# joeyee/Onet

Hardware: AMD Instinct MI355X
Metric: training images/sec (twin 256x256 pass) (higher is better)
Workload: dtype f32

## Files before the change

### onet_amd/_lib.py

```python
from __future__ import annotations

import ctypes
import os
import re

HERE = os.path.dirname(os.path.abspath(__file__))
HEADER = os.path.join(os.path.dirname(HERE), "include", "onet_hip.h")
EVAL_HEADER = os.path.join(os.path.dirname(HERE), "include", "onet_hip_eval.h")
RAGGED_HEADER = os.path.join(os.path.dirname(HERE), "include", "onet_hip_ragged.h")
RAGGED_SPLIT_HEADER = os.path.join(os.path.dirname(HERE), "include", "onet_hip_ragged_split.h")
ANYMAP_HEADER = os.path.join(os.path.dirname(HERE), "include", "onet_hip_anymap.h")
PAIRS_HEADER = os.path.join(os.path.dirname(HERE), "include", "onet_hip_pairs.h")
UPMAP_HEADER = os.path.join(os.path.dirname(HERE), "include", "onet_hip_upmap.h")
SPLIT_PAIRS_HEADER = os.path.join(os.path.dirname(HERE), "include", "onet_hip_split_pairs.h")
OPTIM_HEADER = os.path.join(os.path.dirname(HERE), "include", "onet_hip_optim.h")
LIBPATH = os.environ.get("ONET_HIP_LIB") or os.path.join(HERE, "libonet_hip.so")

_CT = {
    "int": ctypes.c_int,
    "int64_t": ctypes.c_int64,
    "uint64_t": ctypes.c_uint64,
    "float": ctypes.c_float,
    "double": ctypes.c_double,
}


def parse_header(path: str = HEADER):
    src = open(path).read()
    src = re.sub(r"/\*.*?\*/", " ", src, flags=re.S)
    src = re.sub(r"//[^\n]*", " ", src)
# ... 26 lines not shown
_lib = None
_protos = None


def load(build_if_missing: bool = True):
    global _lib, _protos
    if _lib is not None:
        return _lib
    if not os.path.exists(LIBPATH):
        if not build_if_missing:
            raise OnetHipError(f"{LIBPATH} not built; run `python -m onet_amd.build`")
        from . import build as _build
        _build.build()
    lib = ctypes.CDLL(LIBPATH)
    _protos = {}
    for header in (HEADER, EVAL_HEADER, RAGGED_HEADER, RAGGED_SPLIT_HEADER, ANYMAP_HEADER, PAIRS_HEADER, UPMAP_HEADER, SPLIT_PAIRS_HEADER, OPTIM_HEADER):
        protos = parse_header(header)
        for name, (restype, argtypes, _) in protos.items():
            try:
                fn = getattr(lib, name)
            except AttributeError as e:
                raise OnetHipError(f"libonet_hip.so does not export {name} declared in {os.path.basename(header)}") from e
            fn.restype = restype
            fn.argtypes = argtypes
        _protos.update(protos)
    _lib = lib
    return lib


def last_error() -> str:
    return load().onet_last_error().decode()
# ... 16 lines not shown
```

### onet_amd/build.py

```python
import os
import subprocess
import sys

HERE = os.path.dirname(os.path.abspath(__file__))
CSRC = os.path.join(HERE, "csrc")
LIB = os.path.join(HERE, "libonet_hip.so")
SOURCES = ["abi.cpp", "conv_mfma.hip", "conv_wino4.hip", "conv_wino4w.hip", "conv_split.hip", "convt_gemm.hip", "stem.hip", "bn.hip", "spatial.hip", "head_loss.hip", "optim.hip", "evalside.hip", "clutter.hip"]
ARCH = "gfx950"


def _stale():
    if not os.path.exists(LIB):
        return True
    t = os.path.getmtime(LIB)
    deps = [os.path.join(CSRC, f) for f in os.listdir(CSRC) if f.endswith((".hip", ".cpp", ".hpp"))] + \
        [os.path.join(HERE, "..", "include", h) for h in ("onet_hip.h", "onet_hip_eval.h", "onet_hip_ragged.h", "onet_hip_ragged_split.h", "onet_hip_anymap.h", "onet_hip_pairs.h", "onet_hip_upmap.h", "onet_hip_split_pairs.h", "onet_hip_optim.h")]
    return any(os.path.getmtime(d) > t for d in deps)


def build(force=False, verbose=False, variant=None, flags=()):
    lib = LIB if variant is None else os.path.join(HERE, f"libonet_hip_{variant}.so")
    if variant is None and not force and not _stale():
        return LIB
    hipcc = os.environ.get("HIPCC", "/opt/rocm/bin/hipcc")
    objdir = CSRC if variant is None else os.path.join(CSRC, "_" + variant)
    os.makedirs(objdir, exist_ok=True)
    objs = []
    procs = []
    for src in SOURCES:
        obj = os.path.join(objdir, src.rsplit(".", 1)[0] + ".o")
        cmd = [hipcc, "-x", "hip", f"--offload-arch={ARCH}", "-O3", "-fPIC", "-std=c++17", "-Wall",
# ... 26 lines not shown
```

### onet_amd/csrc/conv_mfma.hip

```cpp
#include <algorithm>
#include <cstdlib>
#include "common.hpp"

using namespace onet;

typedef float f32x16 __attribute__((ext_vector_type(16)));

__global__ void pack3x3_kernel(const float* __restrict__ w, float* __restrict__ wf,
                               float* __restrict__ wd, int Cout, int Cin) {
    int64_t n = (int64_t)Cout * Cin * 9;
    for (int64_t i = blockIdx.x * (int64_t)blockDim.x + threadIdx.x; i < n;
         i += (int64_t)gridDim.x * blockDim.x) {
        int t = (int)(i % 9);
        int64_t r = i / 9;
        int ci = (int)(r % Cin), co = (int)(r / Cin);
        float v = w[i];
        if (wf) wf[((int64_t)ci * 9 + t) * Cout + co] = v;
        if (wd) wd[((int64_t)co * 9 + (8 - t)) * Cin + ci] = v;
    }
}

__global__ void packT2x2_kernel(const float* __restrict__ w, float* __restrict__ wf,
                                float* __restrict__ wd, float* __restrict__ wq, int Cin, int Cout) {
    int64_t n = (int64_t)Cin * Cout * 4;
// ... 465 lines not shown
            }
        }
        __syncthreads();
    }
    float* sl = a.slab + (int64_t)ks * TAPS * a.Cout * a.Cin;
    const int ci = ci0 + wn * 32 + l31;
    if (ci < a.Cin) {
#pragma unroll
        for (int t = 0; t < NTAP; ++t) {
#pragma unroll
            for (int r = 0; r < 16; ++r) {
                const int co = co0 + wm * 32 + (r & 3) + 8 * (r >> 2) + 4 * kh;
                if (co < a.Cout) sl[((int64_t)(tg * NTAP + t) * a.Cout + co) * a.Cin + ci] = acc[t][r];
            }
        }
    }
}

__global__ __launch_bounds__(256) void wgrad_reduce_kernel(const float* __restrict__ slab, float* __restrict__ dw,
                                                           int splitK, int taps, int Cout, int Cin, int out_layout,
                                                           int accumulate) {
    __shared__ float red[256];
    const int64_t n = (int64_t)Cout * Cin;
    const int t = blockIdx.y;
    const int64_t i = (int64_t)blockIdx.x * 64 + (threadIdx.x & 63);
    const int g = threadIdx.x >> 6;
    float s = 0.f;
    if (i < n)
        for (int k = g; k < splitK; k += 4) s += slab[((int64_t)k * taps + t) * n + i];
    red[threadIdx.x] = s;
// ... 4 lines not shown
        int64_t o;
        if (out_layout == 0) {
            o = i * taps + t;
        } else {
            const int Ct = Cout / 4, q = co / Ct, cot = co % Ct;
            o = ((int64_t)ci * Ct + cot) * 4 + q;
        }
        dw[o] = accumulate ? dw[o] + s : s;
    }
}

namespace onet {
int launch_wgrad_reduce(const float* slab, float* dw, int splitK, int taps, int Cout, int Cin, int out_layout, int accumulate,
                        hipStream_t st) {
    const int64_t n = (int64_t)Cout * Cin;
    hipLaunchKernelGGL(wgrad_reduce_kernel, dim3((unsigned)cdiv(n, 64), (unsigned)taps), dim3(256), 0, st, slab, dw, splitK,
                       taps, Cout, Cin, out_layout, accumulate);
    return check_launch("wgrad_reduce_kernel");
}
}

constexpr int STEM_ROWS = 32;
template <int CIN, int COG, bool BN = false>
__global__ __launch_bounds__(256) void conv3x3_stem_wgrad_kernel(WgArgs a) {
    constexpr int NV = COG * CIN * 9;
    __shared__ float red[4][NV];
    const int cogs = (a.Cout + COG - 1) / COG;
    const int bandsY = (a.H + STEM_ROWS - 1) / STEM_ROWS;
    const int cg = blockIdx.x % cogs, bb = blockIdx.x / cogs;
    const int b = bb / bandsY, yb = (bb % bandsY) * STEM_ROWS;
// ... 279 lines not shown
    ONET_REQUIRE(twin_B == 0 || 2 * twin_B == B, "conv3x3_stem_wgrad_bn: a twin batch holds twin_B = B / 2 images in memory");
    a.twin_B = twin_B;
    a.twin_bias = twin_bias;
    const int nb = stem_blocks(B, H);
    const int64_t need = (int64_t)nb * 9 * Cout * Cin * 4;
    ONET_REQUIRE(ws_bytes >= need, "conv3x3_stem_wgrad_bn: workspace %lld < %lld bytes", (long long)ws_bytes, (long long)need);
    hipStream_t st = as_stream(stream);
    switch (Cin) {
        case 1: hipLaunchKernelGGL((conv3x3_stem_wgrad_kernel<1, 4, true>), dim3(nb * cdiv(Cout, 4)), dim3(256), 0, st, a); break;
        case 2: hipLaunchKernelGGL((conv3x3_stem_wgrad_kernel<2, 2, true>), dim3(nb * cdiv(Cout, 2)), dim3(256), 0, st, a); break;
        case 3: hipLaunchKernelGGL((conv3x3_stem_wgrad_kernel<3, 2, true>), dim3(nb * cdiv(Cout, 2)), dim3(256), 0, st, a); break;
        default: hipLaunchKernelGGL((conv3x3_stem_wgrad_kernel<4, 1, true>), dim3(nb * cdiv(Cout, 1)), dim3(256), 0, st, a); break;
    }
    int rc = check_launch("conv3x3_stem_wgrad_kernel");
    if (rc) return rc;
    const int64_t n = (int64_t)Cout * Cin;
    hipLaunchKernelGGL(wgrad_reduce_kernel, dim3((unsigned)cdiv(n, 64), 9u), dim3(256), 0, st, (const float*)ws, dw, nb, 9, Cout, Cin, 0, accumulate);
    return check_launch("wgrad_reduce_kernel");
}

int onet_conv_wgrad(const float* x, int64_t x_bs, const float* dz, int64_t dz_bs, float* dw, void* ws,
                    int64_t ws_bytes, int B, int Cin, int Cout, int H, int W, int ks, int out_layout,
                    int accumulate, void* stream) {
    ONET_REQUIRE(x && dz && dw && ws, "conv_wgrad: null pointer");
    ONET_REQUIRE(B > 0 && Cin > 0 && Cout > 0 && H > 0 && W > 0, "conv_wgrad: bad shape");
    ONET_REQUIRE(ks == 1 || ks == 3, "conv_wgrad: ks must be 1 or 3 (got %d)", ks);
    ONET_REQUIRE(out_layout == 0 || (out_layout == 1 && ks == 1 && Cout % 4 == 0), "conv_wgrad: bad out_layout");
    WgArgs a{x, x_bs, dz, dz_bs, (float*)ws, B, Cin, Cout, H, W, cdiv(Cin, 64), cdiv(Cout, 64), 1, 1, 1};
    if (use_stem_wgrad(Cin, ks) && out_layout == 0) {
        const int nb = stem_blocks(B, H);
        const int64_t need = (int64_t)nb * 9 * Cout * Cin * 4;
        ONET_REQUIRE(ws_bytes >= need, "conv_wgrad(stem): workspace %lld < %lld bytes", (long long)ws_bytes, (long long)need);
        hipStream_t st = as_stream(stream);
        switch (Cin) {
            case 1: hipLaunchKernelGGL((conv3x3_stem_wgrad_kernel<1, 4>), dim3(nb * cdiv(Cout, 4)), dim3(256), 0, st, a); break;
            case 2: hipLaunchKernelGGL((conv3x3_stem_wgrad_kernel<2, 2>), dim3(nb * cdiv(Cout, 2)), dim3(256), 0, st, a); break;
            case 3: hipLaunchKernelGGL((conv3x3_stem_wgrad_kernel<3, 2>), dim3(nb * cdiv(Cout, 2)), dim3(256), 0, st, a); break;
            default: hipLaunchKernelGGL((conv3x3_stem_wgrad_kernel<4, 1>), dim3(nb * cdiv(Cout, 1)), dim3(256), 0, st, a); break;
        }
        int rc = check_launch("conv3x3_stem_wgrad_kernel");
        if (rc) return rc;
        const int64_t n = (int64_t)Cout * Cin;
        hipLaunchKernelGGL(wgrad_reduce_kernel, dim3((unsigned)cdiv(n, 64), 9u), dim3(256), 0, st,
                           (const float*)ws, dw, nb, 9, Cout, Cin, 0, accumulate);
        return check_launch("wgrad_reduce_kernel");
    }
    int pw;
    wgrad_plan(B, Cin, Cout, H, W, ks, pw, a.splitK, a.stripsX, a.stripsY);
    const int64_t need = (int64_t)a.splitK * ks * ks * Cout * Cin * 4;
    ONET_REQUIRE(ws_bytes >= need, "conv_wgrad: workspace %lld < %lld bytes", (long long)ws_bytes, (long long)need);
    const int64_t blocks = (int64_t)a.splitK * a.ciTiles * a.coTiles;
    hipStream_t st = as_stream(stream);
    if (ks == 3) {
        if (pw == 32) launch_wgrad<3, 32>(a, blocks, st); else launch_wgrad<3, 16>(a, blocks, st);
    } else {
        if (pw == 32) launch_wgrad<1, 32>(a, blocks, st); else launch_wgrad<1, 16>(a, blocks, st);
    }
    int rc = check_launch("conv_wgrad_kernel");
    if (rc) return rc;
    const int64_t n = (int64_t)Cout * Cin;
    hipLaunchKernelGGL(wgrad_reduce_kernel, dim3((unsigned)cdiv(n, 64), (unsigned)(ks * ks)), dim3(256), 0, st,
                       (const float*)ws, dw, a.splitK, ks * ks, Cout, Cin, out_layout, accumulate);
    return check_launch("wgrad_reduce_kernel");
}

int onet_convT2x2_wgrad(const float* x, int64_t x_bs, const float* dy, int64_t dy_bs, float* dw, void* ws,
                        int64_t ws_bytes, int B, int Cin, int Ct, int h, int w, int Ho, int Wo, int pt, int pl, int operand_bf16,
                        void* stream) {
    ONET_REQUIRE(x && dy && dw && ws, "convT2x2_wgrad: null pointer");
    ONET_REQUIRE(B > 0 && Cin > 0 && Ct > 0 && h > 0 && w > 0, "convT2x2_wgrad: bad shape");
    ONET_REQUIRE(Ct % 64 == 0, "convT2x2_wgrad: Ct must be a multiple of 64 (use onet_space_to_depth2 + onet_conv_wgrad)");
    ONET_REQUIRE(pt >= 0 && pl >= 0 && pt + 2 * h <= Ho && pl + 2 * w <= Wo, "convT2x2_wgrad: window outside plane");
    ONET_REQUIRE(dy_bs >= (int64_t)Ct * Ho * Wo && x_bs >= (int64_t)Cin * h * w, "convT2x2_wgrad: batch stride too small");
    if (convt_gemm_enabled()) {
        const int rc = convt_gemm_wgrad(x, x_bs, dy, dy_bs, dw, ws, ws_bytes, B, Cin, Ct, h, w, Ho, Wo, pt, pl, operand_bf16, as_stream(stream));
        if (rc <= 0) return rc;
    }
    const int Cout = 4 * Ct;
    WgArgs a{x, x_bs, dy, dy_bs, (float*)ws, B, Cin, Cout, h, w, cdiv(Cin, 64), cdiv(Cout, 64), 1, 1, 1, Ct, Ho, Wo, pt, pl};
    int pw;
    wgrad_plan(B, Cin, Cout, h, w, 1, pw, a.splitK, a.stripsX, a.stripsY);
    const int64_t need = (int64_t)a.splitK * Cout * Cin * 4;
    ONET_REQUIRE(ws_bytes >= need, "convT2x2_wgrad: workspace %lld < %lld bytes", (long long)ws_bytes, (long long)need);
    const int64_t blocks = (int64_t)a.splitK * a.ciTiles * a.coTiles;
    hipStream_t st = as_stream(stream);
    if (pw == 32) launch_wgrad<1, 32, true>(a, blocks, st); else launch_wgrad<1, 16, true>(a, blocks, st);
    int rc = check_launch("conv_wgrad_kernel");
    if (rc) return rc;
    const int64_t n = (int64_t)Cout * Cin;
    hipLaunchKernelGGL(wgrad_reduce_kernel, dim3((unsigned)cdiv(n, 64), 1u), dim3(256), 0, st, (const float*)ws, dw,
                       a.splitK, 1, Cout, Cin, 1, 0);
    return check_launch("wgrad_reduce_kernel");
}

}
```

### onet_amd/csrc/conv_split.hip

```cpp
#include <algorithm>
#include <cstdlib>
#include "common.hpp"
#include "../../include/onet_hip_ragged.h"
#include "../../include/onet_hip_ragged_split.h"
#include "../../include/onet_hip_anymap.h"
#include "../../include/onet_hip_pairs.h"
#include "../../include/onet_hip_split_pairs.h"

using namespace onet;

typedef float f32x16 __attribute__((ext_vector_type(16)));
typedef __bf16 bf16x8 __attribute__((ext_vector_type(8)));
typedef __bf16 bf16x2 __attribute__((ext_vector_type(2)));
typedef unsigned int u32x4s __attribute__((ext_vector_type(4)));
typedef float f32x4s __attribute__((ext_vector_type(4)));

namespace {

constexpr unsigned OOB_S = 0x80000000u;

__device__ __forceinline__ __amdgpu_buffer_rsrc_t s_rsrc(const void* base, int64_t bytes) {
    const int n = bytes > 0x7fffffffll ? 0x7fffffff : (int)bytes;
    return __builtin_amdgcn_make_buffer_rsrc(const_cast<void*>(base), 0, n, 0x00020000);
}
// ... 14 lines not shown
    const f16x2 h = {(_Float16)a, (_Float16)b};
    const f16x2 m = {(_Float16)(a - (float)h[0]), (_Float16)(b - (float)h[1])};
    hi = __builtin_bit_cast(unsigned, h);
    mid = __builtin_bit_cast(unsigned, m);
}

__global__ void absmax_slots_kernel(const float* __restrict__ v, int64_t n, unsigned* __restrict__ slots) {
    float m = 0.f;
    for (int64_t i = blockIdx.x * (int64_t)blockDim.x + threadIdx.x; i < n; i += (int64_t)gridDim.x * blockDim.x) m = fmaxf(m, fabsf(v[i]));
#pragma unroll
    for (int o = 32; o > 0; o >>= 1) m = fmaxf(m, __shfl_xor(m, o, 64));
    if ((threadIdx.x & 63) == 0)
        atomicMax(slots + ((blockIdx.x * (blockDim.x >> 6) + (threadIdx.x >> 6)) & (AMAX_SLOTS - 1)) * AMAX_STRIDE, __builtin_bit_cast(unsigned, m));
}

__global__ void pack3x3_split_kernel(const float* __restrict__ w, __bf16* __restrict__ wq, int Cout, int Cin, int which, int f16,
                                     const unsigned* __restrict__ wamax) {
    const int K = which == 0 ? Cin : ((Cout + 15) / 16) * 16, N = which == 0 ? Cout : Cin;
    const int64_t n = (int64_t)K * 9 * N;
    const int nparts = f16 == 2 ? 1 : 2;
    float winv = 1.f;
    const float wscale = f16 == 1 ? amax_scale(amax_read(wamax), true, winv) : 1.f;
    if (blockIdx.x == 0 && threadIdx.x == 0) {
        float* meta = reinterpret_cast<float*>(wq + nparts * n);
        meta[0] = wscale;
        meta[1] = winv;
    }
    for (int64_t i = blockIdx.x * (int64_t)blockDim.x + threadIdx.x; i < n; i += (int64_t)gridDim.x * blockDim.x) {
        const int kc = (int)(i & 7);
        int64_t r = i >> 3;
        const int nn = (int)(r % N);
        r /= N;
        const int half = (int)(r & 1);
        r >>= 1;
        const int t = (int)(r % 9), kg = (int)(r / 9);
        const int k = kg * 16 + half * 8 + kc;
        float v = 0.f;
        if (which == 0) v = w[((int64_t)nn * Cin + k) * 9 + t];
        else if (k < Cout) v = w[((int64_t)k * Cin + nn) * 9 + (8 - t)];
        const int64_t per_chunk_part = (int64_t)9 * 2 * N * 8;
        const int64_t within = i - (int64_t)kg * per_chunk_part;
        if (f16 == 2) {
            wq[(int64_t)kg * per_chunk_part + within] = (__bf16)v;
        } else if (f16) {
            _Float16* wh = reinterpret_cast<_Float16*>(wq);
            const float vs = v * wscale;
            const _Float16 hi = (_Float16)vs;
            wh[((int64_t)kg * 2 + 0) * per_chunk_part + within] = hi;
            wh[((int64_t)kg * 2 + 1) * per_chunk_part + within] = (_Float16)(vs - (float)hi);
        } else {
            const __bf16 hi = (__bf16)v;
            wq[((int64_t)kg * 2 + 0) * per_chunk_part + within] = hi;
            wq[((int64_t)kg * 2 + 1) * per_chunk_part + within] = (__bf16)(v - (float)hi);
        }
    }
}

struct SpArgs {
    const float* x;
    int64_t x_bs;
    const __bf16* wq;
    float* z;
    int64_t z_bs;
    int B, Cin, Cout, H, W, tilesX, tilesY, coTiles;
    float* stats;
    const float* nsave;
    int nimg;
    const unsigned* x_amax;
    int x_always;
// ... 2175 lines not shown
                                    int dgrad_f16, void* stream) {
    ONET_REQUIRE(w && (wq_fwd || wq_dgrad), "conv3x3_split_pack_weights: null pointer");
    ONET_REQUIRE(amax_ws || !(fwd_f16 == 1 || dgrad_f16 == 1), "conv3x3_split_pack_weights: the fp16 packs need the 8 KB magnitude workspace");
    if (fwd_f16 == 1 || dgrad_f16 == 1) {
        (void)hipMemsetAsync(amax_ws, 0, AMAX_SLOTS * AMAX_STRIDE * sizeof(unsigned), as_stream(stream));
        const int64_t nw = (int64_t)Cout * Cin * 9;
        hipLaunchKernelGGL(absmax_slots_kernel, dim3((unsigned)std::min<int64_t>((nw + 1023) / 1024, 1024)), dim3(256), 0, as_stream(stream), w,
                           nw, (unsigned*)amax_ws);
        int rc0 = check_launch("absmax_slots_kernel");
        if (rc0) return rc0;
    }
    ONET_REQUIRE(Cout > 0 && Cin > 0, "conv3x3_split_pack_weights: bad shape");
    ONET_REQUIRE(!wq_fwd || (Cin % 16) == 0, "conv3x3_split_pack_weights: the forward pack needs Cin %% 16 == 0");
    const int64_t n = (int64_t)std::max(Cin, ((Cout + 15) / 16) * 16) * 9 * std::max(Cin, Cout);
    const int blocks = (int)std::min<int64_t>((n + 255) / 256, 8192);
    if (wq_fwd) {
        hipLaunchKernelGGL(pack3x3_split_kernel, dim3(blocks), dim3(256), 0, as_stream(stream), w, (__bf16*)wq_fwd, Cout, Cin, 0, fwd_f16,
                           (const unsigned*)amax_ws);
        int rc = check_launch("pack3x3_split_kernel");
        if (rc) return rc;
    }
    if (wq_dgrad) hipLaunchKernelGGL(pack3x3_split_kernel, dim3(blocks), dim3(256), 0, as_stream(stream), w, (__bf16*)wq_dgrad, Cout, Cin, 1,
                                     dgrad_f16, (const unsigned*)amax_ws);
    return check_launch("pack3x3_split_kernel");
}

int onet_conv3x3_split_fwd(const float* x, int64_t x_bs, const void* wq, int wq_f16, float* z, int64_t z_bs, int B, int Cin, int Cout,
                           int H, int W, void* stream) {
    return split_fwd(x, x_bs, wq, z, z_bs, B, Cin, Cout, H, W, stream, nullptr, wq_f16);
}

int onet_absmax_slots(const float* x, int64_t n, void* slots, void* stream) {
    ONET_REQUIRE(x && slots && n > 0, "absmax_slots: bad args");
    hipLaunchKernelGGL(absmax_slots_kernel, dim3((unsigned)std::min<int64_t>((n + 1023) / 1024, 4096)), dim3(256), 0, as_stream(stream), x, n,
                       (unsigned*)slots);
    return check_launch("absmax_slots_kernel");
}

// ... 522 lines not shown
```

### onet_amd/csrc/convt_gemm.hip

```cpp
#include <algorithm>
#include <cstdlib>
#include "common.hpp"
#include "../../include/onet_hip_ragged.h"
#include "../../include/onet_hip_ragged_split.h"
#include "../../include/onet_hip_upmap.h"

using namespace onet;

typedef float f32x16 __attribute__((ext_vector_type(16)));
typedef float f32x4g __attribute__((ext_vector_type(4)));
typedef float f32x2g __attribute__((ext_vector_type(2)));
typedef int i32x4g __attribute__((ext_vector_type(4)));
typedef __bf16 bf16x8g __attribute__((ext_vector_type(8)));
typedef __bf16 bf16x2g __attribute__((ext_vector_type(2)));
typedef unsigned u32x4g __attribute__((ext_vector_type(4)));

namespace {

__device__ __forceinline__ i32x4g g_rsrc(const void* base, int64_t bytes) {
    const uint64_t p = reinterpret_cast<uint64_t>(base);
    i32x4g r;
    r.x = (int)(p & 0xffffffffu);
    r.y = (int)((p >> 32) & 0xffffu);
    r.z = bytes > 0x7fffffffll ? 0x7fffffff : (int)bytes;
// ... 406 lines not shown

    float* slab = g.out + (int64_t)ks * g.Cin * 4 * g.Ct;
#pragma unroll
    for (int t = 0; t < 2; ++t)
#pragma unroll
        for (int u = 0; u < 2; ++u) {
            const int m = 4 * c0 + wc * 64 + u * 32 + l31;
#pragma unroll
            for (int r = 0; r < 16; ++r) {
                const int ci = ci0 + wr * 64 + t * 32 + (r & 3) + 8 * (r >> 2) + 4 * kh;
                slab[(int64_t)ci * 4 * g.Ct + m] = acc[t][u][r];
            }
        }
}

__global__ __launch_bounds__(256) void convt_wgrad_reduce_kernel(const float* __restrict__ slab, float* __restrict__ dw, int splitK,
                                                                 int64_t n4, int accumulate) {
    const int64_t i = blockIdx.x * (int64_t)blockDim.x + threadIdx.x;
    if (i >= n4) return;
    float4 s = reinterpret_cast<const float4*>(slab)[i];
    for (int k = 1; k < splitK; ++k) {
        const float4 v = reinterpret_cast<const float4*>(slab)[(int64_t)k * n4 + i];
        s.x += v.x; s.y += v.y; s.z += v.z; s.w += v.w;
    }
    if (accumulate) {
        const float4 o = reinterpret_cast<float4*>(dw)[i];
        s.x += o.x; s.y += o.y; s.z += o.z; s.w += o.w;
    }
    reinterpret_cast<float4*>(dw)[i] = s;
}

__global__ __launch_bounds__(256) void convt_dbias_reduce_kernel(const float* __restrict__ part, float* __restrict__ db, int ntiles, int Ct) {
    const int c = blockIdx.x;
    double s = 0.0;
    for (int t = threadIdx.x; t < ntiles; t += 256) s += (double)part[(int64_t)t * Ct + c];
    __shared__ double sh[4];
    double v[1] = {s};
    block_sum_256<double, 1>(v, sh);
    if (threadIdx.x == 0) db[c] = (float)v[0];
}


typedef _Float16 f16x8g __attribute__((ext_vector_type(8)));

struct SArgs {
    const void* wP;
    const void* xP;
    int64_t x_bs;
    const float* bias;
    void* yP;
    int64_t y_bs;
    const unsigned* x_slots;
    const unsigned* y_slots;
    int B, Cin, Ct, h, w, mTiles, nTiles;
// ... 687 lines not shown
    const int64_t hw = (int64_t)h * w;
    if (pt || pl || Ho != 2 * h || Wo != 2 * w || (Cin % 128) || (Ct % 32) || (hw % KP) || (w & 1) || !aligned16(x) || !aligned16(dy) ||
        !aligned16(dw) || (x_bs & 3) || (dy_bs & 3) || (int64_t)Cin * hw * 4 >= (1ll << 31) || (int64_t)Ct * Ho * Wo * 4 >= (1ll << 31))
        return 1;
    GArgs g{x, dy, (float*)ws, nullptr, nullptr, nullptr, 0, x_bs, dy_bs, 0, B, Cin, Ct, h, w, Wo, Ho * Wo, Cin / 128, Ct / 32, 1, 0};
    wgrad_plan(B, Cin, Ct, h, w, g.splitK, g.chunksPerSplit);
    const int64_t n = (int64_t)Cin * 4 * Ct;
    if (ws_bytes < (int64_t)g.splitK * n * 4) return 1;
    const int64_t blocks = (int64_t)g.splitK * g.mTiles * g.nTiles;
    if (prec == 2) hipLaunchKernelGGL(convt_wgrad_gemm_kernel<2>, dim3((unsigned)blocks), dim3(256), 0, st, g);
    else if (prec) hipLaunchKernelGGL(convt_wgrad_gemm_kernel<1>, dim3((unsigned)blocks), dim3(256), 0, st, g);
    else hipLaunchKernelGGL(convt_wgrad_gemm_kernel<0>, dim3((unsigned)blocks), dim3(256), 0, st, g);
    int rc = check_launch("convt_wgrad_gemm_kernel");
    if (rc) return rc;
    hipLaunchKernelGGL(convt_wgrad_reduce_kernel, dim3((unsigned)cdiv(n / 4, 256)), dim3(256), 0, st, (const float*)ws, dw, g.splitK,
                       n / 4, 0);
    return check_launch("convt_wgrad_reduce_kernel");
}

}

static bool wgrad_slots_plan(int B, int Cin, int Ct, int h, int w, int& splitK, int& per) {
    const bool big = (Cin % 256) == 0 && (Ct % 64) == 0;
    const int64_t chunks = (int64_t)B * h * w / SW_CP;
    const int64_t tiles = big ? (int64_t)(Cin / 256) * (Ct / 64) : (int64_t)(Cin / 128) * (Ct / 32);
    int64_t k = std::max<int64_t>(1, ((big ? 256 : 512) + tiles - 1) / tiles);
    k = std::min<int64_t>(k, std::max<int64_t>(1, chunks / (512 / SW_CP)));
    k = std::min<int64_t>(k, std::max<int64_t>(1, (256ll << 20) / ((int64_t)Cin * 4 * Ct * 4)));
    per = (int)((chunks + k - 1) / k);
    splitK = (int)((chunks + per - 1) / per);
    return big;
}

template <int NP, int BIG>
static int launch_wgrad_slots(SWArgs g, hipStream_t st) {
    using C = SwCfg<BIG>;
    const int lds = NP * (C::APL + C::BPL) * C::PXP * 16 * C::NST;
    auto kern = convt_slot_wgrad_kernel<NP, BIG>;
    static PerDeviceOnce once;
    if (once.first()) (void)hipFuncSetAttribute(reinterpret_cast<const void*>(kern), hipFuncAttributeMaxDynamicSharedMemorySize, lds);
    const int64_t blocks = (int64_t)g.splitK * g.mTiles * g.nTiles;
    ONET_REQUIRE(blocks > 0 && blocks < (1ll << 31), "convT2x2_wgrad_slots: grid too large");
    hipLaunchKernelGGL(kern, dim3((unsigned)blocks), dim3(C::NWAVE * 64), lds, st, g);
    return check_launch("convt_slot_wgrad_kernel");
}

extern "C" {

int onet_convT2x2_pack_weights_slots(const float* w, void* wP, void* wdP, void* amax_ws, int Cin, int Ct, int nparts, void* stream) {
    ONET_REQUIRE(w && wP && Cin > 0 && Ct > 0 && (Cin % 8) == 0 && (!wdP || (Ct % 8) == 0) && (nparts == 1 || nparts == 2),
                 "convT2x2_pack_weights_slots: bad args");
    ONET_REQUIRE(nparts == 1 || amax_ws, "convT2x2_pack_weights_slots: the fp16 pack needs the 8 KB magnitude workspace");
    hipStream_t st = as_stream(stream);
    const int64_t n = (int64_t)Cin * 4 * Ct;
    if (nparts == 2) {
        (void)hipMemsetAsync(amax_ws, 0, AMAX_SLOTS * AMAX_STRIDE * sizeof(unsigned), st);
        hipLaunchKernelGGL(convt_absmax_kernel, dim3((unsigned)std::min<int64_t>((n + 1023) / 1024, 1024)), dim3(256), 0, st, w, n, (unsigned*)amax_ws);
        int rc = check_launch("convt_absmax_kernel");
        if (rc) return rc;
    }
    hipLaunchKernelGGL(convt_pack_slots_kernel, dim3((unsigned)std::min<int64_t>(((wdP ? 2 : 1) * n + 255) / 256, 8192)), dim3(256), 0, st, w, wP,
                       wdP, Cin, Ct, nparts, (const unsigned*)amax_ws);
// ... 33 lines not shown
    ONET_REQUIRE(xP_bs >= (int64_t)Cin * hw * nparts / 2 && dyP_bs >= (int64_t)Ct * 4 * hw * nparts / 2, "convT2x2_wgrad_slots: batch stride too small");
    int lw = 0;
    while ((1 << lw) < w) ++lw;
    SWArgs g{xP, xP_bs, dyP, dyP_bs, (float*)ws, nullptr, (const unsigned*)x_amax, (const unsigned*)dy_amax, B, Cin, Ct, h, w, lw, 0, 0, 1, 0};
    const bool big = wgrad_slots_plan(B, Cin, Ct, h, w, g.splitK, g.chunksPerSplit);
    g.mTiles = big ? Cin / 256 : Cin / 128;
    g.nTiles = big ? Ct / 64 : Ct / 32;
    const int64_t n = (int64_t)Cin * 4 * Ct;
    ONET_REQUIRE(ws_bytes >= (int64_t)g.splitK * (n + 4 * Ct) * 4, "convT2x2_wgrad_slots: workspace too small (onet_convT2x2_wgrad_slots_ws_bytes)");
    if (dbias) g.db_part = (float*)ws + (int64_t)g.splitK * n;
    hipStream_t st = as_stream(stream);
    int rc;
    if (nparts == 2) rc = big ? launch_wgrad_slots<2, 1>(g, st) : launch_wgrad_slots<2, 0>(g, st);
    else rc = big ? launch_wgrad_slots<1, 1>(g, st) : launch_wgrad_slots<1, 0>(g, st);
    if (rc) return rc;
    hipLaunchKernelGGL(convt_wgrad_reduce_kernel, dim3((unsigned)cdiv(n / 4, 256)), dim3(256), 0, st, (const float*)ws, dw, g.splitK, n / 4, 0);
    rc = check_launch("convt_wgrad_reduce_kernel");
    if (rc || !dbias) return rc;
    hipLaunchKernelGGL(convt_dbias_reduce_kernel, dim3((unsigned)Ct), dim3(256), 0, st, (const float*)g.db_part, dbias, g.splitK * 4, Ct);
    return check_launch("convt_dbias_reduce_kernel");
}

int onet_convT2x2_fwd_slots(const void* xP, int64_t xP_bs, const void* x_amax, const void* wP, const float* bias, void* yP, int64_t yP_bs,
                            const void* y_amax, int nparts, int B, int Cin, int Ct, int h, int w, void* stream) {
    ONET_REQUIRE(xP && wP && yP && B > 0 && Cin > 0 && Ct > 0 && h > 0 && w > 0 && (nparts == 1 || nparts == 2), "convT2x2_fwd_slots: bad args");
    const int64_t hw = (int64_t)h * w;
    if ((Cin % 32) || Cin < 128 || (Ct % 32) || (hw % 128) || (w & 1) || !aligned16(xP) || !aligned16(wP) || !aligned16(yP) || (xP_bs & 3) || (yP_bs & 3) ||
        (int64_t)Cin * hw * 2 * nparts >= (1ll << 31) || (int64_t)Cin * 4 * Ct * 2 * nparts >= (1ll << 31))
        return 1;
    ONET_REQUIRE(xP_bs >= (int64_t)Cin * hw * nparts / 2 && yP_bs >= (int64_t)Ct * 4 * hw * nparts / 2, "convT2x2_fwd_slots: batch stride too small");
    SArgs g{wP, xP, xP_bs, bias, yP, yP_bs, (const unsigned*)x_amax, (const unsigned*)y_amax, B, Cin, Ct, h, w, (4 * Ct) / 128, (int)(B * hw / 128), 2 * h, 2 * w};
    const int64_t blocks = (int64_t)g.mTiles * g.nTiles;
    ONET_REQUIRE(blocks > 0 && blocks < (1ll << 31), "convT2x2_fwd_slots: grid too large");
    if (nparts == 2) hipLaunchKernelGGL(convt_slot_fwd_kernel<2>, dim3((unsigned)blocks), dim3(256), 0, as_stream(stream), g);
    else hipLaunchKernelGGL(convt_slot_fwd_kernel<1>, dim3((unsigned)blocks), dim3(256), 0, as_stream(stream), g);
// ... 58 lines not shown
```

Before: 585.3.

## Vectorize weight-grad split-K reductions and fuse pack and dbias kernels

```diff
diff --git a/include/onet_hip_wtail.h b/include/onet_hip_wtail.h
--- /dev/null
+++ b/include/onet_hip_wtail.h
@@ -0,0 +1,15 @@
+#ifndef ONET_HIP_WTAIL_H
+#define ONET_HIP_WTAIL_H
+#include <stdint.h>
+#ifdef __cplusplus
+extern "C" {
+#endif
+
+int onet_wgrad_reduce(const float* slab, float* dw, int splitK, int taps, int Cout, int Cin, int out_layout, int accumulate, void* stream);
+int onet_convt_wgrad_reduce(const float* slab, float* dw, int splitK, int64_t n, int accumulate, const float* db_part, float* dbias,
+                            int db_tiles, int Ct, void* stream);
+
+#ifdef __cplusplus
+}
+#endif
+#endif
diff --git a/onet_amd/_lib.py b/onet_amd/_lib.py
--- a/onet_amd/_lib.py
+++ b/onet_amd/_lib.py
@@ -14,6 +14,7 @@
 UPMAP_HEADER = os.path.join(os.path.dirname(HERE), "include", "onet_hip_upmap.h")
 SPLIT_PAIRS_HEADER = os.path.join(os.path.dirname(HERE), "include", "onet_hip_split_pairs.h")
 OPTIM_HEADER = os.path.join(os.path.dirname(HERE), "include", "onet_hip_optim.h")
+WTAIL_HEADER = os.path.join(os.path.dirname(HERE), "include", "onet_hip_wtail.h")
 LIBPATH = os.environ.get("ONET_HIP_LIB") or os.path.join(HERE, "libonet_hip.so")
 
 _CT = {
@@ -70,7 +71,7 @@
         _build.build()
     lib = ctypes.CDLL(LIBPATH)
     _protos = {}
-    for header in (HEADER, EVAL_HEADER, RAGGED_HEADER, RAGGED_SPLIT_HEADER, ANYMAP_HEADER, PAIRS_HEADER, UPMAP_HEADER, SPLIT_PAIRS_HEADER, OPTIM_HEADER):
+    for header in (HEADER, EVAL_HEADER, RAGGED_HEADER, RAGGED_SPLIT_HEADER, ANYMAP_HEADER, PAIRS_HEADER, UPMAP_HEADER, SPLIT_PAIRS_HEADER, OPTIM_HEADER, WTAIL_HEADER):
         protos = parse_header(header)
         for name, (restype, argtypes, _) in protos.items():
             try:
diff --git a/onet_amd/build.py b/onet_amd/build.py
--- a/onet_amd/build.py
+++ b/onet_amd/build.py
@@ -14,7 +14,7 @@
         return True
     t = os.path.getmtime(LIB)
     deps = [os.path.join(CSRC, f) for f in os.listdir(CSRC) if f.endswith((".hip", ".cpp", ".hpp"))] + \
-        [os.path.join(HERE, "..", "include", h) for h in ("onet_hip.h", "onet_hip_eval.h", "onet_hip_ragged.h", "onet_hip_ragged_split.h", "onet_hip_anymap.h", "onet_hip_pairs.h", "onet_hip_upmap.h", "onet_hip_split_pairs.h", "onet_hip_optim.h")]
+        [os.path.join(HERE, "..", "include", h) for h in ("onet_hip.h", "onet_hip_eval.h", "onet_hip_ragged.h", "onet_hip_ragged_split.h", "onet_hip_anymap.h", "onet_hip_pairs.h", "onet_hip_upmap.h", "onet_hip_split_pairs.h", "onet_hip_optim.h", "onet_hip_wtail.h")]
     return any(os.path.getmtime(d) > t for d in deps)
 
 
diff --git a/onet_amd/csrc/conv_mfma.hip b/onet_amd/csrc/conv_mfma.hip
--- a/onet_amd/csrc/conv_mfma.hip
+++ b/onet_amd/csrc/conv_mfma.hip
@@ -503,6 +503,101 @@
                 if (co < a.Cout) sl[((int64_t)(tg * NTAP + t) * a.Cout + co) * a.Cin + ci] = acc[t][r];
             }
         }
+    }
+}
+
+constexpr int WGR_MAX_LANES = 72;
+template <int TAPS, int LAYOUT, int D>
+__global__ __launch_bounds__(4 * WGR_MAX_LANES) void wgrad_reduce_vec_kernel(const float* __restrict__ slab, float* __restrict__ dw,
+                                                                             int splitK, int Cout, int Cin, int accumulate, int leq) {
+    __shared__ float red[4 * WGR_MAX_LANES * 4];
+    static_assert(LAYOUT == 0 || TAPS == 1, "the ConvTranspose2d layout has one tap");
+    const int64_t n = (int64_t)Cout * Cin;
+    const int eq = 1 << leq;
+    const int L = LAYOUT == 0 ? TAPS * eq : 64;
+    const int g = LAYOUT == 0 ? (int)(threadIdx.x >> leq) / TAPS : (int)(threadIdx.x >> 6);
+    const int lane = threadIdx.x - g * L;
+    const int Ct = Cout / 4;
+    int t = 0;
+    int64_t i;
+    bool live;
+    if (LAYOUT == 0) {
+        t = lane >> leq;
+        i = ((int64_t)blockIdx.x * eq + (lane & (eq - 1))) * 4;
+        live = i < n;
+    } else {
+        const int row = lane >> 2, q = row >> 2, cot = blockIdx.y * 4 + (row & 3), ci = blockIdx.x * 16 + (lane & 3) * 4;
+        i = ((int64_t)q * Ct + cot) * Cin + ci;
+        live = cot < Ct && ci < Cin;
+    }
+    float4 s = {0.f, 0.f, 0.f, 0.f};
+    const int R = live ? (splitK - g + 3) >> 2 : 0;
+    if (R > 0) {
+        const int64_t rstride = (int64_t)4 * TAPS * n;
+        const float* p = slab + ((int64_t)g * TAPS + t) * n + i;
+#define ONET_WGR_LD(r) (*reinterpret_cast<const float4*>(p + (int64_t)(r) * rstride))
+#define ONET_WGR_ADD(v) do { s.x += (v).x; s.y += (v).y; s.z += (v).z; s.w += (v).w; } while (0)
+        int r = 0;
+        if (R >= D) {
+            float4 v[D];
+#pragma unroll
+            for (int u = 0; u < D; ++u) {
+                v[u] = ONET_WGR_LD(u);
+                __builtin_amdgcn_sched_barrier(0);
+            }
+            for (; r + 2 * D <= R; r += D) {
+#pragma unroll
+                for (int u = 0; u < D; ++u) {
+                    ONET_WGR_ADD(v[u]);
+                    v[u] = ONET_WGR_LD(r + D + u);
+                    __builtin_amdgcn_sched_barrier(0);
+                }
+            }
+#pragma unroll
+            for (int u = 0; u < D; ++u) ONET_WGR_ADD(v[u]);
+            r += D;
+        }
+        for (; r + 4 <= R; r += 4) {
+            float4 v[4];
+#pragma unroll
+            for (int u = 0; u < 4; ++u) v[u] = ONET_WGR_LD(r + u);
+#pragma unroll
+            for (int u = 0; u < 4; ++u) ONET_WGR_ADD(v[u]);
+        }
+        if (r < R) {
+            const float4 a = ONET_WGR_LD(r);
+            float4 b = a, c = a;
+            if (r + 1 < R) b = ONET_WGR_LD(r + 1);
+            if (r + 2 < R) c = ONET_WGR_LD(r + 2);
+            ONET_WGR_ADD(a);
+            if (r + 1 < R) ONET_WGR_ADD(b);
+            if (r + 2 < R) ONET_WGR_ADD(c);
+        }
+#undef ONET_WGR_ADD
+#undef ONET_WGR_LD
+    }
+    *reinterpret_cast<float4*>(red + (g * L + lane) * 4) = s;
+    __syncthreads();
+    const int j = threadIdx.x;
+    int src;
+    int64_t o;
+    if (LAYOUT == 0) {
+        const int e = j / TAPS, tt = j - e * TAPS;
+        const int64_t e0 = (int64_t)blockIdx.x * eq * 4;
+        live = e0 + e < n;
+        src = tt * eq * 4 + e;
+        o = (e0 + e) * TAPS + tt;
+    } else {
+        const int cil = j >> 4, cotl = (j >> 2) & 3, q = j & 3;
+        const int ci = blockIdx.x * 16 + cil, cot = blockIdx.y * 4 + cotl;
+        live = ci < Cin && cot < Ct;
+        src = ((q * 4 + cotl) * 4 + (cil >> 2)) * 4 + (cil & 3);
+        o = ((int64_t)ci * Ct + cot) * 4 + q;
+    }
+    if (live) {
+        const int gs = L * 4;
+        const float r = (red[src] + red[gs + src]) + (red[2 * gs + src] + red[3 * gs + src]);
+        dw[o] = accumulate ? dw[o] + r : r;
     }
 }
 
@@ -537,6 +632,29 @@
 int launch_wgrad_reduce(const float* slab, float* dw, int splitK, int taps, int Cout, int Cin, int out_layout, int accumulate,
                         hipStream_t st) {
     const int64_t n = (int64_t)Cout * Cin;
+    const bool aligned = (reinterpret_cast<uintptr_t>(slab) & 15) == 0;
+#define ONET_WGR_LAUNCH(TAPS_, LAYOUT_, LEQ_)                                                                                               \
+    do {                                                                                                                                    \
+        if (splitK >= 64) hipLaunchKernelGGL((wgrad_reduce_vec_kernel<TAPS_, LAYOUT_, 16>), grid, blk, 0, st, slab, dw, splitK, Cout, Cin,  \
+                                             accumulate, LEQ_);                                                                             \
+        else hipLaunchKernelGGL((wgrad_reduce_vec_kernel<TAPS_, LAYOUT_, 4>), grid, blk, 0, st, slab, dw, splitK, Cout, Cin, accumulate,    \
+                                LEQ_);                                                                                                      \
+    } while (0)
+    if (aligned && out_layout == 1 && taps == 1 && Cin % 4 == 0 && Cout % 4 == 0) {
+        const dim3 grid((unsigned)cdiv(Cin, 16), (unsigned)cdiv(Cout / 4, 4)), blk(256);
+        ONET_WGR_LAUNCH(1, 1, 2);
+        return check_launch("wgrad_reduce_vec_kernel");
+    }
+    if (aligned && out_layout == 0 && n % 4 == 0 && (taps == 9 || taps == 4 || taps == 1)) {
+        int leq = taps == 9 ? 2 : taps == 4 ? 3 : 5;
+        if (cdiv(n / 4, 2 << leq) >= 512) ++leq;
+        const dim3 grid((unsigned)cdiv(n / 4, 1 << leq)), blk((unsigned)(4 * taps << leq));
+        if (taps == 9) ONET_WGR_LAUNCH(9, 0, leq);
+        else if (taps == 4) ONET_WGR_LAUNCH(4, 0, leq);
+        else ONET_WGR_LAUNCH(1, 0, leq);
+        return check_launch("wgrad_reduce_vec_kernel");
+    }
+#undef ONET_WGR_LAUNCH
     hipLaunchKernelGGL(wgrad_reduce_kernel, dim3((unsigned)cdiv(n, 64), (unsigned)taps), dim3(256), 0, st, slab, dw, splitK,
                        taps, Cout, Cin, out_layout, accumulate);
     return check_launch("wgrad_reduce_kernel");
@@ -846,9 +964,7 @@
     }
     int rc = check_launch("conv3x3_stem_wgrad_kernel");
     if (rc) return rc;
-    const int64_t n = (int64_t)Cout * Cin;
-    hipLaunchKernelGGL(wgrad_reduce_kernel, dim3((unsigned)cdiv(n, 64), 9u), dim3(256), 0, st, (const float*)ws, dw, nb, 9, Cout, Cin, 0, accumulate);
-    return check_launch("wgrad_reduce_kernel");
+    return launch_wgrad_reduce((const float*)ws, dw, nb, 9, Cout, Cin, 0, accumulate, st);
 }
 
 int onet_conv_wgrad(const float* x, int64_t x_bs, const float* dz, int64_t dz_bs, float* dw, void* ws,
@@ -872,10 +988,7 @@
         }
         int rc = check_launch("conv3x3_stem_wgrad_kernel");
         if (rc) return rc;
-        const int64_t n = (int64_t)Cout * Cin;
-        hipLaunchKernelGGL(wgrad_reduce_kernel, dim3((unsigned)cdiv(n, 64), 9u), dim3(256), 0, st,
-                           (const float*)ws, dw, nb, 9, Cout, Cin, 0, accumulate);
-        return check_launch("wgrad_reduce_kernel");
+        return launch_wgrad_reduce((const float*)ws, dw, nb, 9, Cout, Cin, 0, accumulate, st);
     }
     int pw;
     wgrad_plan(B, Cin, Cout, H, W, ks, pw, a.splitK, a.stripsX, a.stripsY);
@@ -890,10 +1003,7 @@
     }
     int rc = check_launch("conv_wgrad_kernel");
     if (rc) return rc;
-    const int64_t n = (int64_t)Cout * Cin;
-    hipLaunchKernelGGL(wgrad_reduce_kernel, dim3((unsigned)cdiv(n, 64), (unsigned)(ks * ks)), dim3(256), 0, st,
-                       (const float*)ws, dw, a.splitK, ks * ks, Cout, Cin, out_layout, accumulate);
-    return check_launch("wgrad_reduce_kernel");
+    return launch_wgrad_reduce((const float*)ws, dw, a.splitK, ks * ks, Cout, Cin, out_layout, accumulate, st);
 }
 
 int onet_convT2x2_wgrad(const float* x, int64_t x_bs, const float* dy, int64_t dy_bs, float* dw, void* ws,
@@ -919,10 +1029,13 @@
     if (pw == 32) launch_wgrad<1, 32, true>(a, blocks, st); else launch_wgrad<1, 16, true>(a, blocks, st);
     int rc = check_launch("conv_wgrad_kernel");
     if (rc) return rc;
-    const int64_t n = (int64_t)Cout * Cin;
-    hipLaunchKernelGGL(wgrad_reduce_kernel, dim3((unsigned)cdiv(n, 64), 1u), dim3(256), 0, st, (const float*)ws, dw,
-                       a.splitK, 1, Cout, Cin, 1, 0);
-    return check_launch("wgrad_reduce_kernel");
-}
-
-}
+    return launch_wgrad_reduce((const float*)ws, dw, a.splitK, 1, Cout, Cin, 1, 0, st);
+}
+
+int onet_wgrad_reduce(const float* slab, float* dw, int splitK, int taps, int Cout, int Cin, int out_layout, int accumulate, void* stream) {
+    ONET_REQUIRE(slab && dw && splitK > 0 && taps > 0 && Cout > 0 && Cin > 0, "wgrad_reduce: bad args");
+    ONET_REQUIRE(out_layout == 0 || (out_layout == 1 && taps == 1 && Cout % 4 == 0), "wgrad_reduce: bad out_layout");
+    return launch_wgrad_reduce(slab, dw, splitK, taps, Cout, Cin, out_layout, accumulate, as_stream(stream));
+}
+
+}
diff --git a/onet_amd/csrc/conv_split.hip b/onet_amd/csrc/conv_split.hip
--- a/onet_amd/csrc/conv_split.hip
+++ b/onet_amd/csrc/conv_split.hip
@@ -52,19 +52,79 @@
         atomicMax(slots + ((blockIdx.x * (blockDim.x >> 6) + (threadIdx.x >> 6)) & (AMAX_SLOTS - 1)) * AMAX_STRIDE, __builtin_bit_cast(unsigned, m));
 }
 
-__global__ void pack3x3_split_kernel(const float* __restrict__ w, __bf16* __restrict__ wq, int Cout, int Cin, int which, int f16,
-                                     const unsigned* __restrict__ wamax) {
-    const int K = which == 0 ? Cin : ((Cout + 15) / 16) * 16, N = which == 0 ? Cout : Cin;
-    const int64_t n = (int64_t)K * 9 * N;
-    const int nparts = f16 == 2 ? 1 : 2;
+__device__ __forceinline__ void pack3x3_store(__bf16* __restrict__ wq, int f16, float wscale, int kg, int64_t per_chunk_part, int64_t within,
+                                              float v) {
+    if (f16 == 2) {
+        wq[(int64_t)kg * per_chunk_part + within] = (__bf16)v;
+    } else if (f16) {
+        _Float16* wh = reinterpret_cast<_Float16*>(wq);
+        const float vs = v * wscale;
+        const _Float16 hi = (_Float16)vs;
+        wh[((int64_t)kg * 2 + 0) * per_chunk_part + within] = hi;
+        wh[((int64_t)kg * 2 + 1) * per_chunk_part + within] = (_Float16)(vs - (float)hi);
+    } else {
+        const __bf16 hi = (__bf16)v;
+        wq[((int64_t)kg * 2 + 0) * per_chunk_part + within] = hi;
+        wq[((int64_t)kg * 2 + 1) * per_chunk_part + within] = (__bf16)(v - (float)hi);
+    }
+}
+
+__global__ void pack3x3_split_kernel(const float* __restrict__ w, __bf16* __restrict__ wq_fwd, __bf16* __restrict__ wq_dgrad, int Cout, int Cin,
+                                     int fwd_f16, int dgrad_f16, const unsigned* __restrict__ wamax) {
+    const int Kd = ((Cout + 15) / 16) * 16;
+    const int64_t n_fwd = (int64_t)Cin * 9 * Cout, n_dgrad = (int64_t)Kd * 9 * Cin;
     float winv = 1.f;
-    const float wscale = f16 == 1 ? amax_scale(amax_read(wamax), true, winv) : 1.f;
+    const float wscale = (fwd_f16 == 1 || dgrad_f16 == 1) ? amax_scale(amax_read(wamax), true, winv) : 1.f;
+    const float fscale = fwd_f16 == 1 ? wscale : 1.f, dscale = dgrad_f16 == 1 ? wscale : 1.f;
     if (blockIdx.x == 0 && threadIdx.x == 0) {
-        float* meta = reinterpret_cast<float*>(wq + nparts * n);
-        meta[0] = wscale;
-        meta[1] = winv;
+        if (wq_fwd) {
+            float* meta = reinterpret_cast<float*>(wq_fwd + (fwd_f16 == 2 ? 1 : 2) * n_fwd);
+            meta[0] = fscale;
+            meta[1] = fwd_f16 == 1 ? winv : 1.f;
+        }
+        if (wq_dgrad) {
+            float* meta = reinterpret_cast<float*>(wq_dgrad + (dgrad_f16 == 2 ? 1 : 2) * n_dgrad);
+            meta[0] = dscale;
+            meta[1] = dgrad_f16 == 1 ? winv : 1.f;
+        }
     }
-    for (int64_t i = blockIdx.x * (int64_t)blockDim.x + threadIdx.x; i < n; i += (int64_t)gridDim.x * blockDim.x) {
+    const int64_t stride = (int64_t)gridDim.x * blockDim.x;
+    if (wq_fwd && wq_dgrad) {
+        const int64_t pcp_f = (int64_t)9 * 2 * Cout * 8, pcp_d = (int64_t)9 * 2 * Cin * 8;
+        const int64_t n_all = n_fwd + (int64_t)(Kd - Cout) * 9 * Cin;
+        for (int64_t i = blockIdx.x * (int64_t)blockDim.x + threadIdx.x; i < n_all; i += stride) {
+            int co, ci, td;
+            float v = 0.f;
+            if (i < n_fwd) {
+                const int kc = (int)(i & 7);
+                int64_t r = i >> 3;
+                co = (int)(r % Cout);
+                r /= Cout;
+                const int half = (int)(r & 1);
+                r >>= 1;
+                const int t = (int)(r % 9), kg = (int)(r / 9);
+                ci = kg * 16 + half * 8 + kc;
+                td = 8 - t;
+                v = w[((int64_t)co * Cin + ci) * 9 + t];
+                pack3x3_store(wq_fwd, fwd_f16, fscale, kg, pcp_f, i - (int64_t)kg * pcp_f, v);
+            } else {
+                int64_t r = i - n_fwd;
+                ci = (int)(r % Cin);
+                r /= Cin;
+                td = (int)(r % 9);
+                co = Cout + (int)(r / 9);
+            }
+            const int64_t within = ((int64_t)(td * 2 + ((co >> 3) & 1)) * Cin + ci) * 8 + (co & 7);
+            pack3x3_store(wq_dgrad, dgrad_f16, dscale, co >> 4, pcp_d, within, v);
+        }
+        return;
+    }
+    const int which = wq_fwd ? 0 : 1, f16 = which == 0 ? fwd_f16 : dgrad_f16;
+    __bf16* wq = which == 0 ? wq_fwd : wq_dgrad;
+    const int N = which == 0 ? Cout : Cin;
+    const int64_t n = which == 0 ? n_fwd : n_dgrad;
+    const float scale = which == 0 ? fscale : dscale;
+    for (int64_t i = blockIdx.x * (int64_t)blockDim.x + threadIdx.x; i < n; i += stride) {
         const int kc = (int)(i & 7);
         int64_t r = i >> 3;
         const int nn = (int)(r % N);
@@ -77,20 +137,7 @@
         if (which == 0) v = w[((int64_t)nn * Cin + k) * 9 + t];
         else if (k < Cout) v = w[((int64_t)k * Cin + nn) * 9 + (8 - t)];
         const int64_t per_chunk_part = (int64_t)9 * 2 * N * 8;
-        const int64_t within = i - (int64_t)kg * per_chunk_part;
-        if (f16 == 2) {
-            wq[(int64_t)kg * per_chunk_part + within] = (__bf16)v;
-        } else if (f16) {
-            _Float16* wh = reinterpret_cast<_Float16*>(wq);
-            const float vs = v * wscale;
-            const _Float16 hi = (_Float16)vs;
-            wh[((int64_t)kg * 2 + 0) * per_chunk_part + within] = hi;
-            wh[((int64_t)kg * 2 + 1) * per_chunk_part + within] = (_Float16)(vs - (float)hi);
-        } else {
-            const __bf16 hi = (__bf16)v;
-            wq[((int64_t)kg * 2 + 0) * per_chunk_part + within] = hi;
-            wq[((int64_t)kg * 2 + 1) * per_chunk_part + within] = (__bf16)(v - (float)hi);
-        }
+        pack3x3_store(wq, f16, scale, kg, per_chunk_part, i - (int64_t)kg * per_chunk_part, v);
     }
 }
 
@@ -2296,14 +2343,8 @@
     ONET_REQUIRE(!wq_fwd || (Cin % 16) == 0, "conv3x3_split_pack_weights: the forward pack needs Cin %% 16 == 0");
     const int64_t n = (int64_t)std::max(Cin, ((Cout + 15) / 16) * 16) * 9 * std::max(Cin, Cout);
     const int blocks = (int)std::min<int64_t>((n + 255) / 256, 8192);
-    if (wq_fwd) {
-        hipLaunchKernelGGL(pack3x3_split_kernel, dim3(blocks), dim3(256), 0, as_stream(stream), w, (__bf16*)wq_fwd, Cout, Cin, 0, fwd_f16,
-                           (const unsigned*)amax_ws);
-        int rc = check_launch("pack3x3_split_kernel");
-        if (rc) return rc;
-    }
-    if (wq_dgrad) hipLaunchKernelGGL(pack3x3_split_kernel, dim3(blocks), dim3(256), 0, as_stream(stream), w, (__bf16*)wq_dgrad, Cout, Cin, 1,
-                                     dgrad_f16, (const unsigned*)amax_ws);
+    hipLaunchKernelGGL(pack3x3_split_kernel, dim3(blocks), dim3(256), 0, as_stream(stream), w, (__bf16*)wq_fwd, (__bf16*)wq_dgrad, Cout, Cin,
+                       fwd_f16, dgrad_f16, (const unsigned*)amax_ws);
     return check_launch("pack3x3_split_kernel");
 }
 
diff --git a/onet_amd/csrc/convt_gemm.hip b/onet_amd/csrc/convt_gemm.hip
--- a/onet_amd/csrc/convt_gemm.hip
+++ b/onet_amd/csrc/convt_gemm.hip
@@ -444,30 +444,48 @@
         }
 }
 
-__global__ __launch_bounds__(256) void convt_wgrad_reduce_kernel(const float* __restrict__ slab, float* __restrict__ dw, int splitK,
-                                                                 int64_t n4, int accumulate) {
-    const int64_t i = blockIdx.x * (int64_t)blockDim.x + threadIdx.x;
-    if (i >= n4) return;
-    float4 s = reinterpret_cast<const float4*>(slab)[i];
-    for (int k = 1; k < splitK; ++k) {
-        const float4 v = reinterpret_cast<const float4*>(slab)[(int64_t)k * n4 + i];
-        s.x += v.x; s.y += v.y; s.z += v.z; s.w += v.w;
-    }
-    if (accumulate) {
-        const float4 o = reinterpret_cast<float4*>(dw)[i];
-        s.x += o.x; s.y += o.y; s.z += o.z; s.w += o.w;
-    }
-    reinterpret_cast<float4*>(dw)[i] = s;
-}
-
-__global__ __launch_bounds__(256) void convt_dbias_reduce_kernel(const float* __restrict__ part, float* __restrict__ db, int ntiles, int Ct) {
-    const int c = blockIdx.x;
+__device__ __forceinline__ void convt_dbias_reduce_block(const float* __restrict__ part, float* __restrict__ db, int ntiles, int Ct, int c) {
     double s = 0.0;
     for (int t = threadIdx.x; t < ntiles; t += 256) s += (double)part[(int64_t)t * Ct + c];
     __shared__ double sh[4];
     double v[1] = {s};
     block_sum_256<double, 1>(v, sh);
     if (threadIdx.x == 0) db[c] = (float)v[0];
+}
+
+__global__ __launch_bounds__(256) void convt_wgrad_reduce_kernel(const float* __restrict__ slab, float* __restrict__ dw, int splitK,
+                                                                 int64_t n4, int accumulate, const float* __restrict__ db_part,
+                                                                 float* __restrict__ db, int db_tiles, int Ct) {
+    const int64_t dw_blocks = (n4 + 255) / 256;
+    if (blockIdx.x >= dw_blocks) {
+        convt_dbias_reduce_block(db_part, db, db_tiles, Ct, (int)(blockIdx.x - dw_blocks));
+        return;
+    }
+    const int64_t i = blockIdx.x * (int64_t)blockDim.x + threadIdx.x;
+    if (i >= n4) return;
+    const float4* p = reinterpret_cast<const float4*>(slab) + i;
+    float4 s = *p;
+    int k = 1;
+    for (; k + 7 < splitK; k += 8) {
+        float4 v[8];
+#pragma unroll
+        for (int u = 0; u < 8; ++u) v[u] = p[(int64_t)(k + u) * n4];
+#pragma unroll
+        for (int u = 0; u < 8; ++u) { s.x += v[u].x; s.y += v[u].y; s.z += v[u].z; s.w += v[u].w; }
+    }
+    for (; k < splitK; ++k) {
+        const float4 v = p[(int64_t)k * n4];
+        s.x += v.x; s.y += v.y; s.z += v.z; s.w += v.w;
+    }
+    if (accumulate) {
+        const float4 o = reinterpret_cast<float4*>(dw)[i];
+        s.x += o.x; s.y += o.y; s.z += o.z; s.w += o.w;
+    }
+    reinterpret_cast<float4*>(dw)[i] = s;
+}
+
+__global__ __launch_bounds__(256) void convt_dbias_reduce_kernel(const float* __restrict__ part, float* __restrict__ db, int ntiles, int Ct) {
+    convt_dbias_reduce_block(part, db, ntiles, Ct, blockIdx.x);
 }
 
 
@@ -1185,7 +1203,7 @@
     int rc = check_launch("convt_wgrad_gemm_kernel");
     if (rc) return rc;
     hipLaunchKernelGGL(convt_wgrad_reduce_kernel, dim3((unsigned)cdiv(n / 4, 256)), dim3(256), 0, st, (const float*)ws, dw, g.splitK,
-                       n / 4, 0);
+                       n / 4, 0, (const float*)nullptr, (float*)nullptr, 0, Ct);
     return check_launch("convt_wgrad_reduce_kernel");
 }
 
@@ -1216,7 +1234,22 @@
     return check_launch("convt_slot_wgrad_kernel");
 }
 
+static int launch_convt_wgrad_reduce(const float* slab, float* dw, int splitK, int64_t n, int accumulate, const float* db_part, float* dbias,
+                                     int db_tiles, int Ct, hipStream_t st) {
+    const int64_t blocks = cdiv(n / 4, 256) + (db_part ? Ct : 0);
+    hipLaunchKernelGGL(convt_wgrad_reduce_kernel, dim3((unsigned)blocks), dim3(256), 0, st, slab, dw, splitK, n / 4, accumulate, db_part, dbias,
+                       db_part ? db_tiles : 0, Ct);
+    return check_launch("convt_wgrad_reduce_kernel");
+}
+
 extern "C" {
+
+int onet_convt_wgrad_reduce(const float* slab, float* dw, int splitK, int64_t n, int accumulate, const float* db_part, float* dbias,
+                            int db_tiles, int Ct, void* stream) {
+    ONET_REQUIRE(slab && dw && splitK > 0 && n > 0 && (n % 4) == 0 && aligned16(slab) && aligned16(dw), "convt_wgrad_reduce: bad args");
+    ONET_REQUIRE(!db_part || (dbias && db_tiles > 0 && Ct > 0), "convt_wgrad_reduce: bad bias rows");
+    return launch_convt_wgrad_reduce(slab, dw, splitK, n, accumulate, db_part, dbias, db_tiles, Ct, as_stream(stream));
+}
 
 int onet_convT2x2_pack_weights_slots(const float* w, void* wP, void* wdP, void* amax_ws, int Cin, int Ct, int nparts, void* stream) {
     ONET_REQUIRE(w && wP && Cin > 0 && Ct > 0 && (Cin % 8) == 0 && (!wdP || (Ct % 8) == 0) && (nparts == 1 || nparts == 2),
@@ -1280,11 +1313,7 @@
     if (nparts == 2) rc = big ? launch_wgrad_slots<2, 1>(g, st) : launch_wgrad_slots<2, 0>(g, st);
     else rc = big ? launch_wgrad_slots<1, 1>(g, st) : launch_wgrad_slots<1, 0>(g, st);
     if (rc) return rc;
-    hipLaunchKernelGGL(convt_wgrad_reduce_kernel, dim3((unsigned)cdiv(n / 4, 256)), dim3(256), 0, st, (const float*)ws, dw, g.splitK, n / 4, 0);
-    rc = check_launch("convt_wgrad_reduce_kernel");
-    if (rc || !dbias) return rc;
-    hipLaunchKernelGGL(convt_dbias_reduce_kernel, dim3((unsigned)Ct), dim3(256), 0, st, (const float*)g.db_part, dbias, g.splitK * 4, Ct);
-    return check_launch("convt_dbias_reduce_kernel");
+    return launch_convt_wgrad_reduce((const float*)ws, dw, g.splitK, n, 0, dbias ? g.db_part : nullptr, dbias, g.splitK * 4, Ct, st);
 }
 
 int onet_convT2x2_fwd_slots(const void* xP, int64_t xP_bs, const void* x_amax, const void* wP, const float* bias, void* yP, int64_t yP_bs,
```

New measurement: 587.7 (median of 6 runs). About the same (+0.4%).
